# Storm-131/MARL-SortingEnv

Measured on AMD Instinct MI355X. Metric: env-steps/sec (random policy) Env_3_Monolith @65k envs, higher is better.
Workload: dtype int32+f64 (integer state/masks, fp64 rewards, f32 observations); 1 GPU; Env_3_Monolith random-policy rollout, 65536 envs per GPU; env_kind=mono, envs_per_gpu=65536, global_envs=65536, max_steps=200, balesize=200, policy=on-device masked-uniform, seed 2024, steps_per_launch=64, outputs=obs f32[K,N,D], mask u8[K,N,A], action i32, reward f32, done u8 per step, parallelism=env-index sharding x1, no data-path collective in the timed region

## Files before the change

### marl-sortingenv_amd/build.py

```python
from __future__ import annotations

import os
import shutil
import subprocess

PKG_DIR = os.path.dirname(os.path.abspath(__file__))
REPO_ROOT = os.path.dirname(PKG_DIR)
SOURCES = [os.path.join(PKG_DIR, "csrc", "mse_lib.hip"), os.path.join(PKG_DIR, "csrc", "mse_policy.hip"),
           os.path.join(PKG_DIR, "csrc", "mse_ppo.hip"), os.path.join(PKG_DIR, "csrc", "mse_episode.hip")]
HEADERS = [os.path.join(PKG_DIR, "csrc", h) for h in ("mse_device.h", "mse_exact.h", "mse_plan.h", "mse_policy_device.h", "mse_policy_pack.h", "mse_policy_stream.h", "mse_ppo_math.h", "mse_episode_math.h")] + \
          [os.path.join(REPO_ROOT, "include", "mse.h")]
LIB_PATH = os.environ.get("MSE_LIB_PATH") or os.path.join(PKG_DIR, "libmse_hip.so")

HIPCC_FLAGS = [
    "-O3", "--offload-arch=gfx950", "-std=c++17", "-fPIC", "-shared",
    "-ffp-contract=off", "-fno-fast-math",
]


def hipcc_path() -> str:
    for cand in (shutil.which("hipcc"), "/opt/rocm/bin/hipcc"):
        if cand and os.path.exists(cand):
            return cand
    raise RuntimeError("hipcc not found: libmse_hip.so cannot be built")


def is_stale() -> bool:
    if not os.path.exists(LIB_PATH):
        return True
    t = os.path.getmtime(LIB_PATH)
    return any(os.path.getmtime(p) > t for p in SOURCES + HEADERS)


def build_library(force: bool = False, verbose: bool = False) -> str:
    if not force and not is_stale():
        return LIB_PATH
    cmd = [hipcc_path(), *HIPCC_FLAGS, "-I", os.path.join(REPO_ROOT, "include"), *SOURCES, "-o", LIB_PATH]
    if verbose:
        print(" ".join(cmd))
    subprocess.run(cmd, check=True)
    return LIB_PATH


WIDETIE_LIB_PATH = os.path.join(PKG_DIR, "libmse_hip_widetie.so")


def build_widetie_library(force: bool = False) -> str:
    if not force and os.path.exists(WIDETIE_LIB_PATH) and \
            all(os.path.getmtime(p) <= os.path.getmtime(WIDETIE_LIB_PATH) for p in SOURCES + HEADERS):
        return WIDETIE_LIB_PATH
    cmd = [hipcc_path(), *HIPCC_FLAGS, "-DMSE_TIE_WINDOW=0x08000000u", "-I", os.path.join(REPO_ROOT, "include"),
           *SOURCES, "-o", WIDETIE_LIB_PATH]
    subprocess.run(cmd, check=True)
    return WIDETIE_LIB_PATH


if __name__ == "__main__":
    print(build_widetie_library(force=True))
    print(build_library(force=True, verbose=True))
```

### marl-sortingenv_amd/csrc/mse_device.h

```cpp
#pragma once

#include <hip/hip_runtime.h>
#include <stdint.h>

#include "mse_exact.h"
#include "mse_policy_stream.h"

namespace mse {

constexpr int kBlock = 256;
constexpr int kGeneratorPeriod = 20;

enum Plane : int {
    PL_RNG_STATE = 0,
    PL_RNG_INC,
    PL_ACC01,
    PL_ACC23,
    PL_CONT_TRUE,
    PL_CONT_FALSE,
    PL_MISC0,
    PL_MISC1,
    PL_MISC2,
    PL_NOISE_STATE,
    PL_NOISE_INC,
    PL_PRESS_STATE,
    PL_PRESS_INC,
    PL_BALE0,
    PL_BALE1, PL_BALE2, PL_BALE3, PL_BALE4,
    PL_SORTRNG_STATE,
// ... 181 lines not shown

__device__ inline Pcg pcg_seed(uint64_t seed)
{
    uint64_t w[4];
    seed_sequence(seed, w);
    Pcg g;
    g.i_hi = (w[2] << 1) | (w[3] >> 63);
    g.i_lo = (w[3] << 1) | 1ull;
    g.s_lo = 0;
    g.s_hi = 0;
    pcg_advance(g);
    uint64_t lo = g.s_lo + w[1];
    g.s_hi = g.s_hi + w[0] + (lo < g.s_lo ? 1ull : 0ull);
    g.s_lo = lo;
    pcg_advance(g);
    return g;
}

__device__ __forceinline__ uint64_t mix64(uint64_t z)
{
    z = (z ^ (z >> 30)) * 0xBF58476D1CE4E5B9ull;
    z = (z ^ (z >> 27)) * 0x94D049BB133111EBull;
    return z ^ (z >> 31);
}

__device__ __forceinline__ int select_kth_bit(uint32_t bits, int k)
{
    uint32_t lo = bits & 0x7FFu;
    int c = __popc(lo);
    bool up = k >= c;
    k = up ? k - c : k;
    bits = up ? bits >> 11 : lo;
    int base = up ? 11 : 0;
    lo = bits & 0x3Fu;
    c = __popc(lo);
    up = k >= c;
    k = up ? k - c : k;
    bits = up ? bits >> 6 : lo;
    base += up ? 6 : 0;
    for (int i = 0; i < k; ++i) bits &= bits - 1u;
    return base + __ffs((int)bits) - 1;
}

#ifdef MSE_TIMELINE
__device__ unsigned long long g_timeline[4 * 8];
struct Timeline {
    unsigned long long last;
    unsigned long long acc[8];
    __device__ __forceinline__ void start()
    {
        for (int k = 0; k < 8; ++k) acc[k] = 0;
        last = __builtin_readcyclecounter();
    }
    __device__ __forceinline__ void mark(int k)
    {
        if (blockIdx.x != 0) return;
        const unsigned long long now = __builtin_readcyclecounter();
        acc[k] += now - last;
        last = now;
    }
    __device__ __forceinline__ void flush(int role) const
    {
        if ((threadIdx.x & 63) == 0 && blockIdx.x == 0)
            for (int k = 0; k < 8; ++k) atomicAdd(&g_timeline[role * 8 + k], acc[k]);
// ... 379 lines not shown
    pcg_affine(g, t[0], t[1], t[2], t[3]);
}

struct RngLocal {
    Pcg &g;
    __device__ __forceinline__ void begin_step() {}
    __device__ __forceinline__ uint32_t next_hi32()
    {
        pcg_advance(g);
        return pcg_output_hi32(g);
    }
    __device__ __forceinline__ uint64_t last_full() const { return pcg_output(g); }
};

constexpr int kRingDepth = 64;
constexpr int kRingMaxPerStep = 31;
typedef __attribute__((address_space(3))) const uint32_t *lds_u32_ptr;
struct RngRing {
    uint32_t lane_addr;
    const uint64_t *jump_tab;
    Pcg start;
    uint32_t p10;
    uint32_t nxt, nxt2;
    uint32_t f_min, f_max;
#ifdef MSE_TIMELINE
    Timeline *tl;
#endif
    __device__ __forceinline__ void open(uint32_t *lring, int el, const uint64_t *jump_table, Env &e)
    {
        lane_addr = (uint32_t)(uintptr_t)(__attribute__((address_space(3))) uint32_t *)(lring + el);
        jump_tab = jump_table;
        start = e.rng;
        p10 = 0;
        nxt = nxt2 = 0;
#ifdef MSE_TIMELINE
        tl = &e.tl;
#endif
        f_min = 0xFFFFFFFFu;
        f_max = 0u;
    }
    __device__ __forceinline__ uint32_t pos() const { return p10 >> 10; }
    __device__ __forceinline__ uint32_t load(uint32_t q10) const
    {
        return *(lds_u32_ptr)(uintptr_t)((q10 & 0xFC00u) | lane_addr);
    }
    __device__ __forceinline__ void begin_step()
    {
        nxt = load(p10);
        nxt2 = load(p10 + 1024u);
        f_min = 0xFFFFFFFFu;
        f_max = 0u;
    }
};

struct RngCounted {
    Pcg g;
    uint32_t count;
    __device__ __forceinline__ void begin_step() {}
    __device__ __forceinline__ uint32_t next_hi32()
    {
        pcg_advance(g);
        ++count;
        return pcg_output_hi32(g);
    }
    __device__ __forceinline__ uint64_t last_full() const { return pcg_output(g); }
};

#ifndef MSE_TIE_HI
#define MSE_TIE_HI 160u
#endif
#ifndef MSE_TIE_WINDOW
#define MSE_TIE_WINDOW (MSE_TIE_HI + 2u)
#endif

template <bool LITERAL, class RNG>
__device__ __forceinline__ void draw_units(RNG &rng, uint32_t &C, int &rem)
{
    while (rem > 0) {
        const uint32_t T = C >> 24;
        const uint32_t r_hi = rng.next_hi32();
        uint32_t flags = 0;
        bool literal = LITERAL;
        if (!LITERAL) {
            const uint64_t prod = mul64_vv(r_hi, T);
            const uint32_t f = (uint32_t)prod;
            const uint32_t v = (uint32_t)(prod >> 32);
            flags = ((__umul24(v, 0x010101u) | 0x00808080u) - C) & 0x00808080u;
            literal = (f + MSE_TIE_HI) < MSE_TIE_WINDOW;
        }
        if (__builtin_expect(literal, 0)) {
            const int sel = choice4_literal(C, rng.last_full());
            flags = sel == 0 ? 0u : (sel == 1 ? 0x00000080u : (sel == 2 ? 0x00008080u : 0x00808080u));
        }
        C += (flags >> 7) + 0xFEFEFEFFu;
        --rem;
    }
}

#define MSE_RING_DRAW(PIN_HI, POUT, OUSE, OLOAD, EXTRA)        \
    "v_perm_b32 %[x], 0, " PIN_HI ", %[sel]\n\t"              \
    "v_add_u16 %[a], 0x400, %[a]\n\t"                         \
    "v_add_u32 %[t], -1, %[t]\n\t"                            \
    "v_sub_u32 %[x], %[x], %[cb]\n\t"                         \
    "v_cmp_ne_u32_e64 %[cm], %[t], %[tend]\n\t"               \
    "v_lshrrev_b32 %[x], 7, %[x]\n\t"                         \
    "ds_read_b32 %[" OLOAD "], %[a]\n\t"                      \
    EXTRA                                                      \
    "s_waitcnt lgkmcnt(1)\n\t"                                \
    "v_and_b32 %[x], 0x10101, %[x]\n\t"                       \
    "v_mad_u64_u32 " POUT ", %[dm], %[" OUSE "], %[t], 0\n\t" \
    "v_add3_u32 %[cb], %[cb], %[x], %[k]\n\t"                 \
    "s_and_b64 exec, exec, %[cm]\n\t"

__device__ __forceinline__ void draw_units_ring(RngRing &rng, uint32_t &C, int &rem)
{
#ifdef MSE_TIMELINE
    rng.tl->mark(2);
#endif
    uint32_t T = C >> 24;
    const uint32_t n_draws = (uint32_t)rem;
    const uint32_t T_end = T - n_draws;
    uint32_t Cb = C - 0x00808080u;
    uint32_t x;
    uint32_t a = ((rng.p10 + 0x400u) & 0xFC00u) | rng.lane_addr;
    uint64_t sv, cm, dm;
    const uint32_t kSel = 0x0C000000u, kK = 0xFEFEFEFFu;
    asm volatile(
        "s_mov_b64 %[sv], exec\n\t"
        "v_cmp_ne_u32 vcc, 0, %[n]\n\t"
        "s_and_b64 exec, exec, vcc\n\t"
        "s_cbranch_execz 3f\n\t"
        "s_waitcnt lgkmcnt(0)\n\t"
        "v_mad_u64_u32 v[124:125], %[dm], %[o0], %[t], 0\n"
        "1:\n\t"
        MSE_RING_DRAW("v125", "v[126:127]", "o1", "o0", "")
        "s_cbranch_execz 2f\n\t"
        MSE_RING_DRAW("v127", "v[124:125]", "o0", "o1",
                      "v_min3_u32 %[mn], %[mn], v124, v126\n\tv_max3_u32 %[mx], %[mx], v124, v126\n\t")
        "s_cbranch_execnz 1b\n"
        "2:\n\t"
        "s_waitcnt lgkmcnt(0)\n\t"
        "s_mov_b64 exec, %[sv]\n\t"
        "v_and_b32 %[x], 1, %[n]\n\t"
        "v_cmp_ne_u32 vcc, 0, %[x]\n\t"
        "s_and_b64 exec, exec, vcc\n\t"
        "v_swap_b32 %[o0], %[o1]\n\t"
        "v_min_u32 %[mn], %[mn], v124\n\t"
        "v_max_u32 %[mx], %[mx], v124\n"
        "3:\n\t"
        "s_mov_b64 exec, %[sv]"
        : [x] "=&v"(x), [a] "+v"(a), [o0] "+v"(rng.nxt), [o1] "+v"(rng.nxt2), [cb] "+v"(Cb),
          [t] "+v"(T), [mn] "+v"(rng.f_min), [mx] "+v"(rng.f_max), [sv] "=&s"(sv), [cm] "=&s"(cm), [dm] "=&s"(dm)
        : [sel] "s"(kSel), [k] "s"(kK), [tend] "v"(T_end), [n] "v"(n_draws)
        : "vcc", "memory", "v124", "v125", "v126", "v127");
    rng.p10 += n_draws << 10;
    C = Cb + 0x00808080u;
    rem = 0;
#ifdef MSE_TIMELINE
    rng.tl->mark(7);
#endif
}

__device__ __forceinline__ void ring_produce(Pcg &g, uint32_t &w, uint32_t count, uint32_t lane_addr)
{
    uint32_t s0 = (uint32_t)g.s_lo, s1 = (uint32_t)(g.s_lo >> 32), s2 = (uint32_t)g.s_hi, s3 = (uint32_t)(g.s_hi >> 32);
    const uint32_t i0 = (uint32_t)g.i_lo, i1 = (uint32_t)(g.i_lo >> 32), i2 = (uint32_t)g.i_hi, i3 = (uint32_t)(g.i_hi >> 32);
    const uint32_t m0 = 0x9FCCF645u, m1 = 0x4385DF64u, m2 = 0x1FC65DA4u, m3 = 0x2360ED05u;
    uint32_t a = ((w << 10) & 0xFC00u) | lane_addr, left = count;
    uint32_t t0, t1, t2, t3, x, y;
    uint64_t sv, cm, dm, cy;
    asm volatile(
        "s_mov_b64 %[sv], exec\n\t"
        "v_cmp_ne_u32 vcc, 0, %[left]\n\t"
        "s_and_b64 exec, exec, vcc\n\t"
        "s_cbranch_execz 3f\n\t"
        "v_mov_b32 v121, 0\n"
        "1:\n\t"
        "v_mad_u64_u32 v[112:113], %[dm], %[s0], %[m0], 0\n\t"
        "v_mul_lo_u32 %[t3], %[s3], %[m0]\n\t"
// ... 111 lines not shown
        "v_alignbit_b32 v96, v96, v97, v95\n\t"
        "v_add_u16 v94, 0x400, %[a]\n\t"
        "v_add_u32 %[left], -1, %[left]\n\t"
        "ds_write_b32 %[a], v124\n\t"
        "v_cmp_ne_u32_e64 %[cm], 0, %[left]\n\t"
        "ds_write_b32 v94, v96\n\t"
        "v_add_u16 %[a], 0x400, v94\n\t"
        "s_and_b64 exec, exec, %[cm]\n\t"
        "s_cbranch_execnz 1b\n"
        "3:\n\t"
        "s_mov_b64 exec, %[sv]"
        : [s0] "+v"(s0), [s1] "+v"(s1), [s2] "+v"(s2), [s3] "+v"(s3), [a] "+v"(a), [left] "+v"(left), [sv] "=&s"(sv),
          [cm] "=&s"(cm), [dm] "=&s"(dm), [cy] "=&s"(cy), [cy2] "=&s"(cy2)
        : [i0] "v"(i0), [i1] "v"(i1), [i2] "v"(i2), [i3] "v"(i3), [j0] "v"(j0), [j1] "v"(j1), [j2] "v"(j2), [j3] "v"(j3),
          [m0] "s"(m0), [m1] "s"(m1), [m2] "s"(m2), [m3] "s"(m3), [n0] "s"(n0), [n1] "s"(n1), [n2] "s"(n2), [n3] "s"(n3)
        : "vcc", "memory", "v90", "v91", "v92", "v93", "v94", "v95", "v96", "v97", "v98", "v99", "v100", "v101", "v102", "v103",
          "v104", "v105", "v106", "v107", "v108", "v109", "v112", "v113", "v114", "v115", "v116", "v117", "v118", "v119", "v120",
          "v121", "v122", "v123", "v124", "v125", "v126", "v127");
    g.s_lo = (uint64_t)s0 | ((uint64_t)s1 << 32);
    g.s_hi = (uint64_t)s2 | ((uint64_t)s3 << 32);
    w += 2u * pairs;
}

__device__ __forceinline__ void draw_units_local(Pcg &g, uint32_t &C, int &rem, uint32_t &f_min, uint32_t &f_max)
{
    uint32_t T = C >> 24;
    const uint32_t n_draws = (uint32_t)rem;
    const uint32_t T_end = T - n_draws;
    uint32_t Cb = C - 0x00808080u;
    uint32_t s0 = (uint32_t)g.s_lo, s1 = (uint32_t)(g.s_lo >> 32), s2 = (uint32_t)g.s_hi, s3 = (uint32_t)(g.s_hi >> 32);
    const uint32_t i0 = (uint32_t)g.i_lo, i1 = (uint32_t)(g.i_lo >> 32), i2 = (uint32_t)g.i_hi, i3 = (uint32_t)(g.i_hi >> 32);
    const uint32_t m0 = 0x9FCCF645u, m1 = 0x4385DF64u, m2 = 0x1FC65DA4u, m3 = 0x2360ED05u;
    const uint32_t kSel = 0x0C000000u, kK = 0xFEFEFEFFu;
    uint32_t t0, t1, t2, t3, x, y;
    uint64_t sv, cm, dm, cy;
    asm volatile(
        "s_mov_b64 %[sv], exec\n\t"
        "v_cmp_ne_u32 vcc, 0, %[n]\n\t"
        "s_and_b64 exec, exec, vcc\n\t"
        "s_cbranch_execz 3f\n\t"
        "v_mov_b32 v121, 0\n"
        "1:\n\t"
        "v_mad_u64_u32 v[112:113], %[dm], %[s0], %[m0], 0\n\t"
        "v_mul_lo_u32 %[t3], %[s3], %[m0]\n\t"
        "v_mul_lo_u32 %[t0], %[s0], %[m3]\n\t"
        "v_mov_b32 v120, v113\n\t"
        "v_mad_u64_u32 v[114:115], %[dm], %[s0], %[m1], v[120:121]\n\t"
        "v_mul_lo_u32 %[t1], %[s1], %[m2]\n\t"
        "v_mul_lo_u32 %[t2], %[s2], %[m1]\n\t"
        "v_mad_u64_u32 v[116:117], %[cy], %[s1], %[m0], v[114:115]\n\t"
        "v_add3_u32 %[t0], %[t0], %[t1], %[t2]\n\t"
        "v_mov_b32 v120, v117\n\t"
        "v_mad_u64_u32 v[118:119], %[dm], %[s0], %[m2], v[120:121]\n\t"
        "v_add_u32 %[t0], %[t0], %[t3]\n\t"
        "v_mad_u64_u32 v[118:119], %[dm], %[s1], %[m1], v[118:119]\n\t"
        "v_mad_u64_u32 v[118:119], %[dm], %[s2], %[m0], v[118:119]\n\t"
        "v_addc_co_u32_e64 %[t0], %[dm], v119, %[t0], %[cy]\n\t"
        "v_add_co_u32 %[s0], vcc, v112, %[i0]\n\t"
        "v_addc_co_u32 %[s1], vcc, v116, %[i1], vcc\n\t"
        "v_addc_co_u32 %[s2], vcc, v118, %[i2], vcc\n\t"
        "v_addc_co_u32 %[s3], vcc, %[t0], %[i3], vcc\n\t"
        "v_xor_b32 %[x], %[s0], %[s2]\n\t"
        "v_xor_b32 %[y], %[s1], %[s3]\n\t"
        "v_lshrrev_b32 %[t1], 26, %[s3]\n\t"
        "v_cmp_gt_i32 vcc, 0, %[s3]\n\t"
        "v_cndmask_b32 %[t2], %[x], %[y], vcc\n\t"
        "v_cndmask_b32 %[t3], %[y], %[x], vcc\n\t"
        "v_alignbit_b32 %[t2], %[t2], %[t3], %[t1]\n\t"
        "v_mad_u64_u32 v[122:123], %[dm], %[t2], %[t], 0\n\t"
        "v_add_u32 %[t], -1, %[t]\n\t"
        "v_perm_b32 %[x], 0, v123, %[sel]\n\t"
        "v_min_u32 %[mn], %[mn], v122\n\t"
        "v_sub_u32 %[x], %[x], %[cb]\n\t"
        "v_max_u32 %[mx], %[mx], v122\n\t"
        "v_lshrrev_b32 %[x], 7, %[x]\n\t"
        "v_cmp_ne_u32_e64 %[cm], %[t], %[tend]\n\t"
        "v_and_b32 %[x], 0x10101, %[x]\n\t"
        "v_add3_u32 %[cb], %[cb], %[x], %[k]\n\t"
        "s_and_b64 exec, exec, %[cm]\n\t"
        "s_cbranch_execnz 1b\n"
        "3:\n\t"
        "s_mov_b64 exec, %[sv]"
        : [s0] "+v"(s0), [s1] "+v"(s1), [s2] "+v"(s2), [s3] "+v"(s3), [cb] "+v"(Cb), [t] "+v"(T), [mn] "+v"(f_min),
          [mx] "+v"(f_max), [t0] "=&v"(t0), [t1] "=&v"(t1), [t2] "=&v"(t2), [t3] "=&v"(t3), [x] "=&v"(x), [y] "=&v"(y),
          [sv] "=&s"(sv), [cm] "=&s"(cm), [dm] "=&s"(dm), [cy] "=&s"(cy)
        : [i0] "v"(i0), [i1] "v"(i1), [i2] "v"(i2), [i3] "v"(i3), [m0] "s"(m0), [m1] "s"(m1), [m2] "s"(m2), [m3] "s"(m3),
          [sel] "s"(kSel), [k] "s"(kK), [tend] "v"(T_end), [n] "v"(n_draws)
        : "vcc", "memory", "v112", "v113", "v114", "v115", "v116", "v117", "v118", "v119", "v120", "v121", "v122", "v123");
    g.s_lo = (uint64_t)s0 | ((uint64_t)s1 << 32);
    g.s_hi = (uint64_t)s2 | ((uint64_t)s3 << 32);
    C = Cb + 0x00808080u;
    rem = 0;
}

template <int I>
__device__ __forceinline__ void station_split(Env &e, uint32_t &C, const double acc_sorter[4], int &rem)
{
    const uint32_t hi_b = (C >> (8 * I)) & 0xFFu;
    const uint32_t lo_b = I == 0 ? 0u : ((C >> (8 * (I > 0 ? I - 1 : 0))) & 0xFFu);
    const uint32_t target = hi_b - lo_b;
    const uint32_t t = (uint32_t)(int)rint((double)target * acc_sorter[I]);
    rem = (int)(target - t);
    C -= t * (0x01010101u << (8 * I));
    e.ct[I] += (int)t;
    e.cf[I] += rem;
}

template <bool LITERAL, int I, class RNG>
__device__ __forceinline__ void station_pair(Env &e, RNG &rng, uint32_t &C, const double acc_sorter[4])
{
    int rem;
    station_split<I>(e, C, acc_sorter, rem);
    const bool early = rem == 0;
    if (early) station_split<I + 1>(e, C, acc_sorter, rem);
// ... 24 lines not shown
    draw_units_ring(rng, C, rem);
    if (!early) {
        station_split<I + 1>(e, C, acc_sorter, rem);
        draw_units_ring(rng, C, rem);
    }
}

template <bool LITERAL>
__device__ __forceinline__ void sort_material(Env &e, RngRing &rng, uint32_t sorting_word, const double acc_sorter[4])
{
    static_assert(!LITERAL, "the ring carries only the upper 32 output bits");
    const uint32_t p10_0 = rng.p10;
    const int ct0 = e.ct[0], ct1 = e.ct[1], ct2 = e.ct[2], ct3 = e.ct[3];
    const int cf0 = e.cf[0], cf1 = e.cf[1], cf2 = e.cf[2], cf3 = e.cf[3];
    const int ce0 = e.ce;
    rng.begin_step();
    uint32_t C = sorting_word * 0x01010101u;
    station_pair_ring<0>(e, rng, C, acc_sorter);
    station_pair_ring<2>(e, rng, C, acc_sorter);
    e.ce += (int)(C >> 24);
#ifdef MSE_ABL_NOTIE
    if (false) {
#else
    if (__builtin_expect(rng.f_min < MSE_TIE_WINDOW - MSE_TIE_HI || rng.f_max >= 0u - MSE_TIE_HI, 0)) {
#endif
        e.ct[0] = ct0; e.ct[1] = ct1; e.ct[2] = ct2; e.ct[3] = ct3;
        e.cf[0] = cf0; e.cf[1] = cf1; e.cf[2] = cf2; e.cf[3] = cf3;
        e.ce = ce0;
        RngCounted exact;
        exact.g = rng.start;
        exact.count = 0;
        pcg_jump(exact.g, p10_0 >> 10, rng.jump_tab);
        sort_material<false>(e, exact, sorting_word, acc_sorter);
        rng.p10 = p10_0 + (exact.count << 10);
    }
}

template <int I>
__device__ __forceinline__ void station_pair_local(Env &e, Pcg &g, uint32_t &C, const double acc_sorter[4],
                                                   uint32_t &f_min, uint32_t &f_max)
{
    int rem;
    station_split<I>(e, C, acc_sorter, rem);
    const bool early = rem == 0;
    if (early) station_split<I + 1>(e, C, acc_sorter, rem);
    draw_units_local(g, C, rem, f_min, f_max);
    if (!early) {
        station_split<I + 1>(e, C, acc_sorter, rem);
        draw_units_local(g, C, rem, f_min, f_max);
    }
}

__device__ __forceinline__ void sort_material_local_fast(Env &e, Pcg &g, uint32_t sorting_word, const double acc_sorter[4])
{
    const Pcg g0 = g;
    const int ct0 = e.ct[0], ct1 = e.ct[1], ct2 = e.ct[2], ct3 = e.ct[3];
    const int cf0 = e.cf[0], cf1 = e.cf[1], cf2 = e.cf[2], cf3 = e.cf[3];
    const int ce0 = e.ce;
    uint32_t f_min = 0xFFFFFFFFu, f_max = 0u;
    uint32_t C = sorting_word * 0x01010101u;
    station_pair_local<0>(e, g, C, acc_sorter, f_min, f_max);
    station_pair_local<2>(e, g, C, acc_sorter, f_min, f_max);
    e.ce += (int)(C >> 24);
    if (__builtin_expect(f_min < MSE_TIE_WINDOW - MSE_TIE_HI || f_max >= 0u - MSE_TIE_HI, 0)) {
        e.ct[0] = ct0; e.ct[1] = ct1; e.ct[2] = ct2; e.ct[3] = ct3;
        e.cf[0] = cf0; e.cf[1] = cf1; e.cf[2] = cf2; e.cf[3] = cf3;
        e.ce = ce0;
        RngCounted exact;
        exact.g = g0;
        exact.count = 0;
        sort_material<false>(e, exact, sorting_word, acc_sorter);
        g = exact.g;
    }
}

template <bool LITERAL>
__device__ __forceinline__ void sort_material(Env &e, RngLocal &rng, uint32_t sorting_word, const double acc_sorter[4])
{
    if (LITERAL) sort_material<true, RngLocal>(e, rng, sorting_word, acc_sorter);
    else sort_material_local_fast(e, rng.g, sorting_word, acc_sorter);
}

__device__ __forceinline__ uint32_t press_next32(Env &e)
{
    if (e.press_has) {
        e.press_has = 0;
        return e.press_uint;
// ... 798 lines not shown
```

### marl-sortingenv_amd/csrc/mse_lib.hip

```cpp
#include "mse_device.h"
#include "mse_plan.h"
#include "mse_policy_device.h"

#include "mse.h"

#include <cmath>
#include <cstdio>
#include <cstdlib>
#include <cstring>
#include <memory>
#include <new>
#include <string>
#include <type_traits>
#include <vector>

using namespace mse;

extern __shared__ uint4 mse_dyn_lds[];

template <int KIND>
struct LdsLayout {
    static constexpr int D = Dims<KIND>::D, A = Dims<KIND>::A;
    static constexpr int obs_bytes = kBlock * D * 4;
    static constexpr int mask_bytes = (kBlock * A + 15) / 16 * 16;
// ... 200 lines not shown
struct RolloutLayout {
    static constexpr int D = Dims<KIND>::D;
    static constexpr int tile_bytes = (kBlock / 2 * D * 4 + 15) / 16 * 16;
    static constexpr int bale_offset = tile_bytes;
    static constexpr int bale_bytes = 5 * 3 * kBlock * 4;
    static constexpr int noise_offset = bale_offset + bale_bytes;
    static constexpr int noise_bytes = NOISE ? kBlock * 16 : 0;
    static constexpr int table_offset = noise_offset + noise_bytes;
};

template <bool GEN = false, class BALES = BaleRef>
__device__ __forceinline__ void auto_reset_env(Env &e, const Params &P, const Tables &tb, const BALES &bales, int k[4])
{
    e.gen2 = unseeded_gen2(e);
    if (GEN) unseeded_generator(e);
    e.episode += 1u;
    reset_episode_state(e, tb.cst);
    if (P.track_bales) clear_bales(bales);
#pragma unroll
    for (int m = 0; m < 4; ++m) k[m] = 101;
}

template <int KIND, bool GEN = false>
__device__ __forceinline__ int policy_action(const Env &e, uint32_t cur, const Tables &tb, uint32_t flags,
                                             uint32_t pkey, uint64_t t)
{
    if (flags & MSE_ROLLOUT_RULE_BASED) {
        return rule_based_action<KIND>(e, Stage<GEN>::rule_mode(e.st_in, tb));
    }
    const uint32_t rr = mse_policy_word(pkey, t);
    if (flags & MSE_STEP_UNMASKED) return (int)(((uint64_t)rr * (uint32_t)Dims<KIND>::A) >> 32);
    const uint32_t cnt = (uint32_t)__popc(cur);
    return select_kth_bit(cur, (int)(((uint64_t)rr * cnt) >> 32));
}

template <int KIND, bool NOISE, bool LITERAL, bool TRACE = false, bool GEN = false>
__global__ __launch_bounds__(kBlock) void k_step(Params P, uint4 *__restrict__ planes,
                                                 const uint32_t *__restrict__ table_image,
                                                 const int *__restrict__ action, const int *__restrict__ sort_mode,
                                                 uint32_t flags, float *__restrict__ obs_out,
                                                 float *__restrict__ reward_out, double *__restrict__ reward64_out,
                                                 uint8_t *__restrict__ done_out, uint8_t *__restrict__ mask_out,
                                                 float *__restrict__ terminal_obs_out,
                                                 unsigned long long *__restrict__ err_count,
                                                 double *__restrict__ trace_rec = nullptr, long long trace_env = -1)
{
    constexpr int D = Dims<KIND>::D, A = Dims<KIND>::A;
    uint8_t *lds = reinterpret_cast<uint8_t *>(mse_dyn_lds);
    uint32_t *ltab = reinterpret_cast<uint32_t *>(lds + LdsLayout<KIND>::table_offset_step);
    const int tid = threadIdx.x;
    const long long row0 = (long long)blockIdx.x * kBlock;
    const long long i = row0 + tid;
    const bool live = i < P.n;
    const BaleRef bales{planes + (long long)PL_BALE0 * P.n_pad + i, P.n_pad};
    float o[D];
    uint32_t mbits = 0;
// ... 98 lines not shown
    const bool live = i < P.n;
    long long rem = P.n - row0;
    const int n_valid = rem >= kBlock ? kBlock : (rem > 0 ? (int)rem : 0);

    const BaleRefCompact bales{lbale + tid, kBlock};
    if (P.track_bales) {
#pragma unroll
        for (int m = 0; m < 5; ++m) bales.store(m, planes[(long long)(PL_BALE0 + m) * P.n_pad + i]);
    }
    load_tables_to_lds(ltab, table_image, GEN ? P.table_words : P.off_jump, tid);
    const Tables tb = tables_at(ltab, P);

    Env e;
    int sm = -1;
    if (live) {
        load_env<KIND, NOISE>(e, planes, P, i);
        if (GEN) load_gen(e, planes, P, i);
        if (KIND == 2 && sort_mode != nullptr) sm = sort_mode[i];
    }
    __builtin_amdgcn_s_waitcnt(0x0F70);
    uint32_t cur_mask = live ? action_mask_bits<KIND>(e, P) : 1u;
    const uint32_t pkey = mse_policy_key(policy_seed, (uint64_t)(P.index_offset + i));
    if (NOISE && live) lnoise[tid] = pack_u64x2(e.noise.i_lo, e.noise.i_hi);

    for (int s = 0; s < k_steps; ++s) {
        float o[D];
#pragma unroll
        for (int j = 0; j < D; ++j) o[j] = 0.0f;
        uint32_t mbits = 0;
        const long long srow = (long long)s * P.n + row0;
        if (live) {
            if (NOISE) {
                const uint4 q = lnoise[tid];
                e.noise.i_lo = u64_of(q.x, q.y);
                e.noise.i_hi = u64_of(q.z, q.w);
            }
            int a = policy_action<KIND, GEN>(e, cur_mask, tb, flags, pkey, policy_t0 + (uint64_t)s);
            int k[4];
            StepResult r = env_step<KIND, NOISE, LITERAL, false, GEN, BaleRefCompact>(e, P, tb, a, sm, flags, bales, k, o);
            if (__builtin_expect(r.done != 0, 0)) {
                auto_reset_env<GEN, BaleRefCompact>(e, P, tb, bales, k);
                env_obs<KIND, GEN>(e, P, tb, k, o);
            }
            mbits = action_mask_bits<KIND>(e, P);
            cur_mask = mbits;
            if (actions_out != nullptr) __builtin_nontemporal_store(a, &actions_out[(long long)s * P.n + i]);
            if (reward_out != nullptr) __builtin_nontemporal_store((float)r.reward, &reward_out[(long long)s * P.n + i]);
            if (done_out != nullptr) __builtin_nontemporal_store((uint8_t)r.done, &done_out[(long long)s * P.n + i]);
        }
        stage_and_store_halves<KIND>(lds, o, mbits, obs_out ? obs_out + srow * D : nullptr,
                                     mask_out ? mask_out + srow * A : nullptr, n_valid, tid);
    }
    if (live) {
        store_env<KIND, NOISE>(e, planes, P, i, false);
        if (GEN) store_gen(e, planes, P, i);
    }
    if (P.track_bales) {
#pragma unroll
        for (int m = 0; m < 5; ++m) planes[(long long)(PL_BALE0 + m) * P.n_pad + i] = bales.load(m);
    }
}

constexpr int kPoEnvs = 256;
constexpr int kPoThreads = 2 * kPoEnvs;
enum : int { kSnapCt = 0, kSnapCf = 4, kSnapCe = 8, kSnapLpa = 9, kSnapStatus = 10, kSnapAction = 11, kSnapMask = 12, kSnapAcc = 13 };
constexpr int snap_word_count(bool noise, bool acc64) { return kSnapAcc + (noise ? (acc64 ? 8 : 4) : 0); }

template <int KIND, bool NOISE>
struct PoLayout {
    static constexpr int D = Dims<KIND>::D, A = Dims<KIND>::A;
    static constexpr int snap_words = snap_word_count(NOISE, true);
    static constexpr int obs_bytes = kPoEnvs * D * 4;
// ... 31 lines not shown
        TableCopy<kPoThreads, 2> tc;
        tc.issue(table_image, P.table_words, tid);
        tc.commit(ltab, table_image, P.table_words, tid);
    }
    __syncthreads();
    const Tables tb = tables_at(ltab, P);

    if (!observer) {
        __builtin_amdgcn_s_setprio(3);
        const BaleRef bales{lbale + el, kPoEnvs};
        if (P.track_bales) {
#pragma unroll
            for (int m = 0; m < 5; ++m) lbale[m * kPoEnvs + el] = planes[(long long)(PL_BALE0 + m) * P.n_pad + i];
        }
        Env e;
        int sm = -1;
        if (live) {
            load_env<KIND, NOISE>(e, planes, P, i);
            if (KIND == 2 && sort_mode != nullptr) sm = sort_mode[i];
        }
        __builtin_amdgcn_s_waitcnt(0x0F70);
        uint32_t cur_mask = live ? action_mask_bits<KIND>(e, P) : 1u;
        const uint32_t pkey = mse_policy_key(policy_seed, (uint64_t)(P.index_offset + i));
        for (int s = 0; s < k_steps; ++s) {
            if (live) {
                const int a = policy_action<KIND>(e, cur_mask, tb, flags, pkey, policy_t0 + (uint64_t)s);
                Snap sn;
                RngLocal rng{e.rng};
                env_dynamics<KIND, NOISE, LITERAL>(e, rng, P, tb, a, sm, flags, bales, sn);
                if (__builtin_expect(sn.done != 0, 0)) {
                    int kdummy[4];
                    auto_reset_env(e, P, tb, bales, kdummy);
                }
                const uint32_t mbits = action_mask_bits<KIND>(e, P);
                cur_mask = mbits;
                uint32_t *w = lsnap + (s & 1) * SW * kPoEnvs + el;
#pragma unroll
                for (int m = 0; m < 4; ++m) {
                    w[(kSnapCt + m) * kPoEnvs] = (uint32_t)sn.ct[m];
                    w[(kSnapCf + m) * kPoEnvs] = (uint32_t)sn.cf[m];
                }
                w[kSnapCe * kPoEnvs] = (uint32_t)sn.ce;
                w[kSnapLpa * kPoEnvs] = (uint32_t)sn.lpa;
                w[kSnapStatus * kPoEnvs] = pack_snap_status(sn);
                w[kSnapAction * kPoEnvs] = (uint32_t)a;
                w[kSnapMask * kPoEnvs] = mbits;
                if (NOISE) {
#pragma unroll
                    for (int m = 0; m < 4; ++m) {
                        w[(kSnapAcc + 2 * m) * kPoEnvs] = (uint32_t)__double2loint(sn.acc[m]);
                        w[(kSnapAcc + 2 * m + 1) * kPoEnvs] = (uint32_t)__double2hiint(sn.acc[m]);
                    }
                }
            }
            lds_barrier_all();
        }
        if (live) store_env<KIND, NOISE>(e, planes, P, i, false);
        if (P.track_bales) {
#pragma unroll
            for (int m = 0; m < 5; ++m) planes[(long long)(PL_BALE0 + m) * P.n_pad + i] = lbale[m * kPoEnvs + el];
        }
    } else {
        long long rem = P.n - row0;
        const int n_valid_block = rem >= kPoEnvs ? kPoEnvs : (rem > 0 ? (int)rem : 0);
        float o[D];
#pragma unroll
        for (int j = 0; j < D; ++j) o[j] = 0.0f;
        for (int s = 0; s < k_steps; ++s) {
            lds_barrier_all();
            const uint32_t *w = lsnap + (s & 1) * SW * kPoEnvs + el;
            Snap sn;
#pragma unroll
            for (int m = 0; m < 4; ++m) {
                sn.ct[m] = (int)w[(kSnapCt + m) * kPoEnvs];
                sn.cf[m] = (int)w[(kSnapCf + m) * kPoEnvs];
            }
            sn.ce = (int)w[kSnapCe * kPoEnvs];
// ... 187 lines not shown
            uint32_t w2 = (uint32_t)P.ring_worst;
            ring_produce(g, w2, (uint32_t)P.ring_worst,
                         (uint32_t)(uintptr_t)(__attribute__((address_space(3))) uint32_t *)(lring + el));
        }
        tc.commit(ltab, table_image, P.table_words, tid);
    }
    MSE_TL(edge, 0);

    if (role == 2) {
        rng_server_role(P, planes, tb, i, live, k_steps, lring, lpos, el, k_steps >= kRingTwoHalvesFrom);
    } else if (role == 0) {
        __builtin_amdgcn_s_setprio(3);
        const BaleRef bales{lbale + el, kPoEnvs};
        if (P.track_bales) {
#pragma unroll
            for (int m = 0; m < 5; ++m) lbale[m * kPoEnvs + el] = planes[(long long)(PL_BALE0 + m) * P.n_pad + i];
        }
        __builtin_amdgcn_s_waitcnt(0x0F70);
        RngRing rng;
        rng.open(lring, el, tb.jump, e);
        uint32_t cur_mask = action_mask_bits<KIND>(e, P);
        const uint32_t pkey = mse_policy_key(policy_seed, (uint64_t)(P.index_offset + i));
        lpos[el] = 0;
        MSE_TL(edge, 1);
        lds_barrier_all();
        MSE_TL(edge, 2);
#ifdef MSE_TIMELINE
        e.tl.start();
#endif
        for (int s = 0; s < k_steps; ++s) {
            {
                const int a = policy_action<KIND>(e, cur_mask, tb, flags, pkey, policy_t0 + (uint64_t)s);
                MSE_TL(e.tl, 0);
                Snap sn;
                env_dynamics<KIND, NOISE, false>(e, rng, P, tb, a, sm, flags, bales, sn);
                uint32_t *w = lsnap + (s & 1) * SW * kPoEnvs + el;
#pragma unroll
                for (int m = 0; m < 4; ++m) {
                    w[(kSnapCt + m) * kPoEnvs] = (uint32_t)sn.ct[m];
                    w[(kSnapCf + m) * kPoEnvs] = (uint32_t)sn.cf[m];
                }
                w[kSnapCe * kPoEnvs] = (uint32_t)sn.ce;
                w[kSnapLpa * kPoEnvs] = (uint32_t)sn.lpa;
                w[kSnapStatus * kPoEnvs] = pack_snap_status(sn);
                w[kSnapAction * kPoEnvs] = (uint32_t)a;
                if (NOISE) {
#pragma unroll
                    for (int m = 0; m < 4; ++m) w[(kSnapAcc + m) * kPoEnvs] = __float_as_uint((float)sn.acc[m]);
                }
                if (__builtin_expect(sn.done != 0, 0)) {
                    int kdummy[4];
                    auto_reset_env(e, P, tb, bales, kdummy);
                }
                const uint32_t mbits = action_mask_bits<KIND>(e, P);
                cur_mask = mbits;
                w[kSnapMask * kPoEnvs] = mbits;
                lpos[el] = rng.pos();
            }
            MSE_TLB(e.tl, 5);
            lds_barrier_all();
            MSE_TLB(e.tl, 6);
        }
#ifdef MSE_TIMELINE
        e.tl.flush(0);
#endif
        MSE_TL(edge, 3);
        if (live) {
            store_env<KIND, NOISE>(e, planes, P, i, false, false);
        }
        if (P.track_bales && live) {
#pragma unroll
            for (int m = 0; m < 5; ++m) planes[(long long)(PL_BALE0 + m) * P.n_pad + i] = lbale[m * kPoEnvs + el];
        }
        MSE_TL(edge, 5);
#ifdef MSE_TIMELINE
        edge.flush(3);
#endif
    } else {
        long long rem = P.n - row0;
        const int n_valid_block = rem >= kPoEnvs ? kPoEnvs : (rem > 0 ? (int)rem : 0);
// ... 851 lines not shown
    if (P.gen_mode) {
        load_gen(e, planes, P, i);
        update_environment<true>(e, P);
        press_obs<true>(e, P, tb, o);
    } else {
        update_environment<false>(e, P);
        press_obs<false>(e, P, tb, o);
    }
#pragma unroll
    for (int j = 0; j < 16; ++j) obs_out[i * 16 + j] = o[j];
}

template <int KIND>
__global__ __launch_bounds__(kBlock) void k_sample(Params P, const uint4 *__restrict__ planes,
                                                   const uint32_t *__restrict__ table_image, uint32_t flags,
                                                   uint64_t policy_seed, uint64_t policy_t, int *__restrict__ action_out)
{
    const long long i = (long long)blockIdx.x * kBlock + threadIdx.x;
    if (i >= P.n) return;
    const Tables tb = tables_at(table_image, P);
    Env e;
    load_env<KIND, false>(e, planes, P, i);
    const uint32_t key = mse_policy_key(policy_seed, (uint64_t)(P.index_offset + i));
    action_out[i] = P.gen_mode ? policy_action<KIND, true>(e, action_mask_bits<KIND>(e, P), tb, flags, key, policy_t)
                               : policy_action<KIND, false>(e, action_mask_bits<KIND>(e, P), tb, flags, key, policy_t);
}

__global__ __launch_bounds__(kBlock) void k_model_actions(Params P, uint4 *__restrict__ planes, uint32_t flags,
                                                          int *__restrict__ action_out)
{
    const long long i = (long long)blockIdx.x * kBlock + threadIdx.x;
    if (i >= P.n) return;
    Env e;
    load_env<1, false>(e, planes, P, i);
    Rng32 srt, prs;
    {
        const uint4 a = planes[(long long)PL_SORTRNG_STATE * P.n_pad + i], b = planes[(long long)PL_SORTRNG_INC * P.n_pad + i];
        const uint4 x = planes[(long long)PL_SORTRNG_AUX * P.n_pad + i];
        srt.g.s_lo = (uint64_t)a.x | ((uint64_t)a.y << 32);
        srt.g.s_hi = (uint64_t)a.z | ((uint64_t)a.w << 32);
        srt.g.i_lo = (uint64_t)b.x | ((uint64_t)b.y << 32);
        srt.g.i_hi = (uint64_t)b.z | ((uint64_t)b.w << 32);
        srt.uinteger = x.x;
        srt.has = (int)x.y;
    }
    prs.g = e.press;
    prs.uinteger = e.press_uint;
    prs.has = e.press_has;
// ... 1048 lines not shown
```

Before: 20.74 billion env-steps/s.

## Fold tie offset into mad, drop f_max tracking, precompute policy words

The tie-detection offset is folded into the v_mad_u64_u32 addend, so a single min check replaces the min/max pair. This removes the max tracking instructions from the inner unit-draw loops in both the ring and local RNG paths. The v_perm selector constant and flag masks are reworked to match, covering all four bytes. The policy random word for the next step is now computed ahead, overlapping with the store and barrier, and the loop in select_kth_bit is replaced by a branchless multiply/popcount trick. These change delicate bit arithmetic and risk subtle correctness shifts in tie handling.

```diff
diff --git a/marl-sortingenv_amd/build.py b/marl-sortingenv_amd/build.py
--- a/marl-sortingenv_amd/build.py
+++ b/marl-sortingenv_amd/build.py
@@ -8,7 +8,7 @@
 REPO_ROOT = os.path.dirname(PKG_DIR)
 SOURCES = [os.path.join(PKG_DIR, "csrc", "mse_lib.hip"), os.path.join(PKG_DIR, "csrc", "mse_policy.hip"),
            os.path.join(PKG_DIR, "csrc", "mse_ppo.hip"), os.path.join(PKG_DIR, "csrc", "mse_episode.hip")]
-HEADERS = [os.path.join(PKG_DIR, "csrc", h) for h in ("mse_device.h", "mse_exact.h", "mse_plan.h", "mse_policy_device.h", "mse_policy_pack.h", "mse_policy_stream.h", "mse_ppo_math.h", "mse_episode_math.h")] + \
+HEADERS = [os.path.join(PKG_DIR, "csrc", h) for h in ("mse_device.h", "mse_exact.h", "mse_plan.h", "mse_policy_device.h", "mse_policy_pack.h", "mse_policy_stream.h", "mse_select.h", "mse_ppo_math.h", "mse_episode_math.h")] + \
           [os.path.join(REPO_ROOT, "include", "mse.h")]
 LIB_PATH = os.environ.get("MSE_LIB_PATH") or os.path.join(PKG_DIR, "libmse_hip.so")
 
@@ -49,7 +49,7 @@
     if not force and os.path.exists(WIDETIE_LIB_PATH) and \
             all(os.path.getmtime(p) <= os.path.getmtime(WIDETIE_LIB_PATH) for p in SOURCES + HEADERS):
         return WIDETIE_LIB_PATH
-    cmd = [hipcc_path(), *HIPCC_FLAGS, "-DMSE_TIE_WINDOW=0x08000000u", "-I", os.path.join(REPO_ROOT, "include"),
+    cmd = [hipcc_path(), *HIPCC_FLAGS, "-DMSE_TIE_HI=0x04000000u", "-DMSE_TIE_WINDOW=0x08000000u", "-I", os.path.join(REPO_ROOT, "include"),
            *SOURCES, "-o", WIDETIE_LIB_PATH]
     subprocess.run(cmd, check=True)
     return WIDETIE_LIB_PATH
diff --git a/marl-sortingenv_amd/csrc/mse_device.h b/marl-sortingenv_amd/csrc/mse_device.h
--- a/marl-sortingenv_amd/csrc/mse_device.h
+++ b/marl-sortingenv_amd/csrc/mse_device.h
@@ -5,6 +5,7 @@
 
 #include "mse_exact.h"
 #include "mse_policy_stream.h"
+#include "mse_select.h"
 
 namespace mse {
 
@@ -232,24 +233,6 @@
     z = (z ^ (z >> 30)) * 0xBF58476D1CE4E5B9ull;
     z = (z ^ (z >> 27)) * 0x94D049BB133111EBull;
     return z ^ (z >> 31);
-}
-
-__device__ __forceinline__ int select_kth_bit(uint32_t bits, int k)
-{
-    uint32_t lo = bits & 0x7FFu;
-    int c = __popc(lo);
-    bool up = k >= c;
-    k = up ? k - c : k;
-    bits = up ? bits >> 11 : lo;
-    int base = up ? 11 : 0;
-    lo = bits & 0x3Fu;
-    c = __popc(lo);
-    up = k >= c;
-    k = up ? k - c : k;
-    bits = up ? bits >> 6 : lo;
-    base += up ? 6 : 0;
-    for (int i = 0; i < k; ++i) bits &= bits - 1u;
-    return base + __ffs((int)bits) - 1;
 }
 
 #ifdef MSE_TIMELINE
@@ -675,7 +658,7 @@
     Pcg start;
     uint32_t p10;
     uint32_t nxt, nxt2;
-    uint32_t f_min, f_max;
+    uint32_t f_min;
 #ifdef MSE_TIMELINE
     Timeline *tl;
 #endif
@@ -690,7 +673,6 @@
         tl = &e.tl;
 #endif
         f_min = 0xFFFFFFFFu;
-        f_max = 0u;
     }
     __device__ __forceinline__ uint32_t pos() const { return p10 >> 10; }
     __device__ __forceinline__ uint32_t load(uint32_t q10) const
@@ -702,7 +684,6 @@
         nxt = load(p10);
         nxt2 = load(p10 + 1024u);
         f_min = 0xFFFFFFFFu;
-        f_max = 0u;
     }
 };
 
@@ -735,11 +716,11 @@
         uint32_t flags = 0;
         bool literal = LITERAL;
         if (!LITERAL) {
-            const uint64_t prod = mul64_vv(r_hi, T);
-            const uint32_t f = (uint32_t)prod;
+            const uint64_t prod = mul64_vv(r_hi, T) + MSE_TIE_HI;
+            const uint32_t f_hi = (uint32_t)prod;
             const uint32_t v = (uint32_t)(prod >> 32);
             flags = ((__umul24(v, 0x010101u) | 0x00808080u) - C) & 0x00808080u;
-            literal = (f + MSE_TIE_HI) < MSE_TIE_WINDOW;
+            literal = f_hi < MSE_TIE_WINDOW;
         }
         if (__builtin_expect(literal, 0)) {
             const int sel = choice4_literal(C, rng.last_full());
@@ -751,7 +732,7 @@
 }
 
 #define MSE_RING_DRAW(PIN_HI, POUT, OUSE, OLOAD, EXTRA)        \
-    "v_perm_b32 %[x], 0, " PIN_HI ", %[sel]\n\t"              \
+    "v_perm_b32 %[x], 0, " PIN_HI ", 0\n\t"                   \
     "v_add_u16 %[a], 0x400, %[a]\n\t"                         \
     "v_add_u32 %[t], -1, %[t]\n\t"                            \
     "v_sub_u32 %[x], %[x], %[cb]\n\t"                         \
@@ -760,8 +741,8 @@
     "ds_read_b32 %[" OLOAD "], %[a]\n\t"                      \
     EXTRA                                                      \
     "s_waitcnt lgkmcnt(1)\n\t"                                \
-    "v_and_b32 %[x], 0x10101, %[x]\n\t"                       \
-    "v_mad_u64_u32 " POUT ", %[dm], %[" OUSE "], %[t], 0\n\t" \
+    "v_and_b32 %[x], 0x1010101, %[x]\n\t"                     \
+    "v_mad_u64_u32 " POUT ", %[dm], %[" OUSE "], %[t], %[hi]\n\t" \
     "v_add3_u32 %[cb], %[cb], %[x], %[k]\n\t"                 \
     "s_and_b64 exec, exec, %[cm]\n\t"
 
@@ -773,23 +754,23 @@
     uint32_t T = C >> 24;
     const uint32_t n_draws = (uint32_t)rem;
     const uint32_t T_end = T - n_draws;
-    uint32_t Cb = C - 0x00808080u;
+    uint32_t Cb = C - 0x80808080u;
     uint32_t x;
     uint32_t a = ((rng.p10 + 0x400u) & 0xFC00u) | rng.lane_addr;
     uint64_t sv, cm, dm;
-    const uint32_t kSel = 0x0C000000u, kK = 0xFEFEFEFFu;
+    const uint32_t kK = 0xFEFEFEFFu;
+    const uint64_t kTieHi = MSE_TIE_HI;
     asm volatile(
         "s_mov_b64 %[sv], exec\n\t"
         "v_cmp_ne_u32 vcc, 0, %[n]\n\t"
         "s_and_b64 exec, exec, vcc\n\t"
         "s_cbranch_execz 3f\n\t"
         "s_waitcnt lgkmcnt(0)\n\t"
-        "v_mad_u64_u32 v[124:125], %[dm], %[o0], %[t], 0\n"
+        "v_mad_u64_u32 v[124:125], %[dm], %[o0], %[t], %[hi]\n"
         "1:\n\t"
         MSE_RING_DRAW("v125", "v[126:127]", "o1", "o0", "")
         "s_cbranch_execz 2f\n\t"
-        MSE_RING_DRAW("v127", "v[124:125]", "o0", "o1",
-                      "v_min3_u32 %[mn], %[mn], v124, v126\n\tv_max3_u32 %[mx], %[mx], v124, v126\n\t")
+        MSE_RING_DRAW("v127", "v[124:125]", "o0", "o1", "v_min3_u32 %[mn], %[mn], v124, v126\n\t")
         "s_cbranch_execnz 1b\n"
         "2:\n\t"
         "s_waitcnt lgkmcnt(0)\n\t"
@@ -798,16 +779,15 @@
         "v_cmp_ne_u32 vcc, 0, %[x]\n\t"
         "s_and_b64 exec, exec, vcc\n\t"
         "v_swap_b32 %[o0], %[o1]\n\t"
-        "v_min_u32 %[mn], %[mn], v124\n\t"
-        "v_max_u32 %[mx], %[mx], v124\n"
+        "v_min_u32 %[mn], %[mn], v124\n"
         "3:\n\t"
         "s_mov_b64 exec, %[sv]"
         : [x] "=&v"(x), [a] "+v"(a), [o0] "+v"(rng.nxt), [o1] "+v"(rng.nxt2), [cb] "+v"(Cb),
-          [t] "+v"(T), [mn] "+v"(rng.f_min), [mx] "+v"(rng.f_max), [sv] "=&s"(sv), [cm] "=&s"(cm), [dm] "=&s"(dm)
-        : [sel] "s"(kSel), [k] "s"(kK), [tend] "v"(T_end), [n] "v"(n_draws)
+          [t] "+v"(T), [mn] "+v"(rng.f_min), [sv] "=&s"(sv), [cm] "=&s"(cm), [dm] "=&s"(dm)
+        : [k] "s"(kK), [hi] "s"(kTieHi), [tend] "v"(T_end), [n] "v"(n_draws)
         : "vcc", "memory", "v124", "v125", "v126", "v127");
     rng.p10 += n_draws << 10;
-    C = Cb + 0x00808080u;
+    C = Cb + 0x80808080u;
     rem = 0;
 #ifdef MSE_TIMELINE
     rng.tl->mark(7);
@@ -965,16 +945,17 @@
     w += 2u * pairs;
 }
 
-__device__ __forceinline__ void draw_units_local(Pcg &g, uint32_t &C, int &rem, uint32_t &f_min, uint32_t &f_max)
+__device__ __forceinline__ void draw_units_local(Pcg &g, uint32_t &C, int &rem, uint32_t &f_min)
 {
     uint32_t T = C >> 24;
     const uint32_t n_draws = (uint32_t)rem;
     const uint32_t T_end = T - n_draws;
-    uint32_t Cb = C - 0x00808080u;
+    uint32_t Cb = C - 0x80808080u;
     uint32_t s0 = (uint32_t)g.s_lo, s1 = (uint32_t)(g.s_lo >> 32), s2 = (uint32_t)g.s_hi, s3 = (uint32_t)(g.s_hi >> 32);
     const uint32_t i0 = (uint32_t)g.i_lo, i1 = (uint32_t)(g.i_lo >> 32), i2 = (uint32_t)g.i_hi, i3 = (uint32_t)(g.i_hi >> 32);
     const uint32_t m0 = 0x9FCCF645u, m1 = 0x4385DF64u, m2 = 0x1FC65DA4u, m3 = 0x2360ED05u;
-    const uint32_t kSel = 0x0C000000u, kK = 0xFEFEFEFFu;
+    const uint32_t kK = 0xFEFEFEFFu;
+    const uint64_t kTieHi = MSE_TIE_HI;
     uint32_t t0, t1, t2, t3, x, y;
     uint64_t sv, cm, dm, cy;
     asm volatile(
@@ -1010,29 +991,28 @@
         "v_cndmask_b32 %[t2], %[x], %[y], vcc\n\t"
         "v_cndmask_b32 %[t3], %[y], %[x], vcc\n\t"
         "v_alignbit_b32 %[t2], %[t2], %[t3], %[t1]\n\t"
-        "v_mad_u64_u32 v[122:123], %[dm], %[t2], %[t], 0\n\t"
+        "v_mad_u64_u32 v[122:123], %[dm], %[t2], %[t], %[hi]\n\t"
         "v_add_u32 %[t], -1, %[t]\n\t"
-        "v_perm_b32 %[x], 0, v123, %[sel]\n\t"
+        "v_perm_b32 %[x], 0, v123, 0\n\t"
         "v_min_u32 %[mn], %[mn], v122\n\t"
         "v_sub_u32 %[x], %[x], %[cb]\n\t"
-        "v_max_u32 %[mx], %[mx], v122\n\t"
         "v_lshrrev_b32 %[x], 7, %[x]\n\t"
         "v_cmp_ne_u32_e64 %[cm], %[t], %[tend]\n\t"
-        "v_and_b32 %[x], 0x10101, %[x]\n\t"
+        "v_and_b32 %[x], 0x1010101, %[x]\n\t"
         "v_add3_u32 %[cb], %[cb], %[x], %[k]\n\t"
         "s_and_b64 exec, exec, %[cm]\n\t"
         "s_cbranch_execnz 1b\n"
         "3:\n\t"
         "s_mov_b64 exec, %[sv]"
         : [s0] "+v"(s0), [s1] "+v"(s1), [s2] "+v"(s2), [s3] "+v"(s3), [cb] "+v"(Cb), [t] "+v"(T), [mn] "+v"(f_min),
-          [mx] "+v"(f_max), [t0] "=&v"(t0), [t1] "=&v"(t1), [t2] "=&v"(t2), [t3] "=&v"(t3), [x] "=&v"(x), [y] "=&v"(y),
+          [t0] "=&v"(t0), [t1] "=&v"(t1), [t2] "=&v"(t2), [t3] "=&v"(t3), [x] "=&v"(x), [y] "=&v"(y),
           [sv] "=&s"(sv), [cm] "=&s"(cm), [dm] "=&s"(dm), [cy] "=&s"(cy)
         : [i0] "v"(i0), [i1] "v"(i1), [i2] "v"(i2), [i3] "v"(i3), [m0] "s"(m0), [m1] "s"(m1), [m2] "s"(m2), [m3] "s"(m3),
-          [sel] "s"(kSel), [k] "s"(kK), [tend] "v"(T_end), [n] "v"(n_draws)
+          [k] "s"(kK), [hi] "s"(kTieHi), [tend] "v"(T_end), [n] "v"(n_draws)
         : "vcc", "memory", "v112", "v113", "v114", "v115", "v116", "v117", "v118", "v119", "v120", "v121", "v122", "v123");
     g.s_lo = (uint64_t)s0 | ((uint64_t)s1 << 32);
     g.s_hi = (uint64_t)s2 | ((uint64_t)s3 << 32);
-    C = Cb + 0x00808080u;
+    C = Cb + 0x80808080u;
     rem = 0;
 }
 
@@ -1103,7 +1083,7 @@
 #ifdef MSE_ABL_NOTIE
     if (false) {
 #else
-    if (__builtin_expect(rng.f_min < MSE_TIE_WINDOW - MSE_TIE_HI || rng.f_max >= 0u - MSE_TIE_HI, 0)) {
+    if (__builtin_expect(rng.f_min < MSE_TIE_WINDOW, 0)) {
 #endif
         e.ct[0] = ct0; e.ct[1] = ct1; e.ct[2] = ct2; e.ct[3] = ct3;
         e.cf[0] = cf0; e.cf[1] = cf1; e.cf[2] = cf2; e.cf[3] = cf3;
@@ -1119,16 +1099,16 @@
 
 template <int I>
 __device__ __forceinline__ void station_pair_local(Env &e, Pcg &g, uint32_t &C, const double acc_sorter[4],
-                                                   uint32_t &f_min, uint32_t &f_max)
+                                                   uint32_t &f_min)
 {
     int rem;
     station_split<I>(e, C, acc_sorter, rem);
     const bool early = rem == 0;
     if (early) station_split<I + 1>(e, C, acc_sorter, rem);
-    draw_units_local(g, C, rem, f_min, f_max);
+    draw_units_local(g, C, rem, f_min);
     if (!early) {
         station_split<I + 1>(e, C, acc_sorter, rem);
-        draw_units_local(g, C, rem, f_min, f_max);
+        draw_units_local(g, C, rem, f_min);
     }
 }
 
@@ -1138,12 +1118,12 @@
     const int ct0 = e.ct[0], ct1 = e.ct[1], ct2 = e.ct[2], ct3 = e.ct[3];
     const int cf0 = e.cf[0], cf1 = e.cf[1], cf2 = e.cf[2], cf3 = e.cf[3];
     const int ce0 = e.ce;
-    uint32_t f_min = 0xFFFFFFFFu, f_max = 0u;
+    uint32_t f_min = 0xFFFFFFFFu;
     uint32_t C = sorting_word * 0x01010101u;
-    station_pair_local<0>(e, g, C, acc_sorter, f_min, f_max);
-    station_pair_local<2>(e, g, C, acc_sorter, f_min, f_max);
+    station_pair_local<0>(e, g, C, acc_sorter, f_min);
+    station_pair_local<2>(e, g, C, acc_sorter, f_min);
     e.ce += (int)(C >> 24);
-    if (__builtin_expect(f_min < MSE_TIE_WINDOW - MSE_TIE_HI || f_max >= 0u - MSE_TIE_HI, 0)) {
+    if (__builtin_expect(f_min < MSE_TIE_WINDOW, 0)) {
         e.ct[0] = ct0; e.ct[1] = ct1; e.ct[2] = ct2; e.ct[3] = ct3;
         e.cf[0] = cf0; e.cf[1] = cf1; e.cf[2] = cf2; e.cf[3] = cf3;
         e.ce = ce0;
diff --git a/marl-sortingenv_amd/csrc/mse_lib.hip b/marl-sortingenv_amd/csrc/mse_lib.hip
--- a/marl-sortingenv_amd/csrc/mse_lib.hip
+++ b/marl-sortingenv_amd/csrc/mse_lib.hip
@@ -246,16 +246,21 @@
 }
 
 template <int KIND, bool GEN = false>
-__device__ __forceinline__ int policy_action(const Env &e, uint32_t cur, const Tables &tb, uint32_t flags,
-                                             uint32_t pkey, uint64_t t)
+__device__ __forceinline__ int policy_action(const Env &e, uint32_t cur, const Tables &tb, uint32_t flags, uint32_t rr)
 {
     if (flags & MSE_ROLLOUT_RULE_BASED) {
         return rule_based_action<KIND>(e, Stage<GEN>::rule_mode(e.st_in, tb));
     }
-    const uint32_t rr = mse_policy_word(pkey, t);
     if (flags & MSE_STEP_UNMASKED) return (int)(((uint64_t)rr * (uint32_t)Dims<KIND>::A) >> 32);
     const uint32_t cnt = (uint32_t)__popc(cur);
     return select_kth_bit(cur, (int)(((uint64_t)rr * cnt) >> 32));
+}
+
+__device__ __forceinline__ uint32_t next_policy_word(uint32_t pkey, uint64_t t)
+{
+    uint32_t w = mse_policy_word(pkey, t);
+    asm volatile("" : "+v"(w));
+    return w;
 }
 
 template <int KIND, bool NOISE, bool LITERAL, bool TRACE = false, bool GEN = false>
@@ -400,6 +405,7 @@
     uint32_t cur_mask = live ? action_mask_bits<KIND>(e, P) : 1u;
     const uint32_t pkey = mse_policy_key(policy_seed, (uint64_t)(P.index_offset + i));
     if (NOISE && live) lnoise[tid] = pack_u64x2(e.noise.i_lo, e.noise.i_hi);
+    uint32_t pword = mse_policy_word(pkey, policy_t0);
 
     for (int s = 0; s < k_steps; ++s) {
         float o[D];
@@ -413,7 +419,7 @@
                 e.noise.i_lo = u64_of(q.x, q.y);
                 e.noise.i_hi = u64_of(q.z, q.w);
             }
-            int a = policy_action<KIND, GEN>(e, cur_mask, tb, flags, pkey, policy_t0 + (uint64_t)s);
+            int a = policy_action<KIND, GEN>(e, cur_mask, tb, flags, pword);
             int k[4];
             StepResult r = env_step<KIND, NOISE, LITERAL, false, GEN, BaleRefCompact>(e, P, tb, a, sm, flags, bales, k, o);
             if (__builtin_expect(r.done != 0, 0)) {
@@ -426,6 +432,7 @@
             if (reward_out != nullptr) __builtin_nontemporal_store((float)r.reward, &reward_out[(long long)s * P.n + i]);
             if (done_out != nullptr) __builtin_nontemporal_store((uint8_t)r.done, &done_out[(long long)s * P.n + i]);
         }
+        pword = next_policy_word(pkey, policy_t0 + (uint64_t)s + 1u);
         stage_and_store_halves<KIND>(lds, o, mbits, obs_out ? obs_out + srow * D : nullptr,
                                      mask_out ? mask_out + srow * A : nullptr, n_valid, tid);
     }
@@ -503,9 +510,10 @@
         __builtin_amdgcn_s_waitcnt(0x0F70);
         uint32_t cur_mask = live ? action_mask_bits<KIND>(e, P) : 1u;
         const uint32_t pkey = mse_policy_key(policy_seed, (uint64_t)(P.index_offset + i));
+        uint32_t pword = mse_policy_word(pkey, policy_t0);
         for (int s = 0; s < k_steps; ++s) {
             if (live) {
-                const int a = policy_action<KIND>(e, cur_mask, tb, flags, pkey, policy_t0 + (uint64_t)s);
+                const int a = policy_action<KIND>(e, cur_mask, tb, flags, pword);
                 Snap sn;
                 RngLocal rng{e.rng};
                 env_dynamics<KIND, NOISE, LITERAL>(e, rng, P, tb, a, sm, flags, bales, sn);
@@ -534,6 +542,7 @@
                     }
                 }
             }
+            pword = next_policy_word(pkey, policy_t0 + (uint64_t)s + 1u);
             lds_barrier_all();
         }
         if (live) store_env<KIND, NOISE>(e, planes, P, i, false);
@@ -767,6 +776,7 @@
         uint32_t cur_mask = action_mask_bits<KIND>(e, P);
         const uint32_t pkey = mse_policy_key(policy_seed, (uint64_t)(P.index_offset + i));
         lpos[el] = 0;
+        uint32_t pword = mse_policy_word(pkey, policy_t0);
         MSE_TL(edge, 1);
         lds_barrier_all();
         MSE_TL(edge, 2);
@@ -775,7 +785,7 @@
 #endif
         for (int s = 0; s < k_steps; ++s) {
             {
-                const int a = policy_action<KIND>(e, cur_mask, tb, flags, pkey, policy_t0 + (uint64_t)s);
+                const int a = policy_action<KIND>(e, cur_mask, tb, flags, pword);
                 MSE_TL(e.tl, 0);
                 Snap sn;
                 env_dynamics<KIND, NOISE, false>(e, rng, P, tb, a, sm, flags, bales, sn);
@@ -801,6 +811,7 @@
                 cur_mask = mbits;
                 w[kSnapMask * kPoEnvs] = mbits;
                 lpos[el] = rng.pos();
+                pword = next_policy_word(pkey, policy_t0 + (uint64_t)s + 1u);
             }
             MSE_TLB(e.tl, 5);
             lds_barrier_all();
@@ -1698,8 +1709,9 @@
     Env e;
     load_env<KIND, false>(e, planes, P, i);
     const uint32_t key = mse_policy_key(policy_seed, (uint64_t)(P.index_offset + i));
-    action_out[i] = P.gen_mode ? policy_action<KIND, true>(e, action_mask_bits<KIND>(e, P), tb, flags, key, policy_t)
-                               : policy_action<KIND, false>(e, action_mask_bits<KIND>(e, P), tb, flags, key, policy_t);
+    const uint32_t word = mse_policy_word(key, policy_t);
+    action_out[i] = P.gen_mode ? policy_action<KIND, true>(e, action_mask_bits<KIND>(e, P), tb, flags, word)
+                               : policy_action<KIND, false>(e, action_mask_bits<KIND>(e, P), tb, flags, word);
 }
 
 __global__ __launch_bounds__(kBlock) void k_model_actions(Params P, uint4 *__restrict__ planes, uint32_t flags,
diff --git a/marl-sortingenv_amd/csrc/mse_select.h b/marl-sortingenv_amd/csrc/mse_select.h
--- /dev/null
+++ b/marl-sortingenv_amd/csrc/mse_select.h
@@ -0,0 +1,35 @@
+#pragma once
+
+#include <stdint.h>
+
+#if defined(__HIPCC__)
+#define MSE_SEL_HD __host__ __device__ __forceinline__
+#if defined(__HIP_DEVICE_COMPILE__)
+#define MSE_SEL_POPC(x) __popc(x)
+#else
+#define MSE_SEL_POPC(x) __builtin_popcount(x)
+#endif
+#else
+#define MSE_SEL_HD static inline
+#define MSE_SEL_POPC(x) __builtin_popcount(x)
+#endif
+
+MSE_SEL_HD int select_kth_bit(uint32_t bits, int k)
+{
+    uint32_t lo = bits & 0x7FFu;
+    int c = MSE_SEL_POPC(lo);
+    bool up = k >= c;
+    k = up ? k - c : k;
+    bits = up ? bits >> 11 : lo;
+    int base = up ? 11 : 0;
+    lo = bits & 0x3Fu;
+    c = MSE_SEL_POPC(lo);
+    up = k >= c;
+    k = up ? k - c : k;
+    bits = up ? bits >> 6 : lo;
+    base += up ? 6 : 0;
+    const uint32_t kOnes = 0x10204081u, kFlags = 0x81020408u;
+    const uint32_t s = (bits * 0x01041041u) & kOnes;
+    const uint32_t t = ((uint32_t)k - s) * kOnes + kFlags;
+    return base + MSE_SEL_POPC(t & kFlags);
+}
```

Measured after the change: 21.15 billion env-steps/s, median of 6. 2.0% higher.
